# octavian-ganea/equidock_public

Measured on NVIDIA H100. Metric: protein_pairs_per_sec_iegmn_fwd_kabsch, higher is better.
Workload: dtype f32

## Files before the change

### equidock_public_b200/csrc/edge_stage_tc.cu

```cuda
#include "tc_common.cuh"

namespace eqd {
#define TC_WGS 3
#define TC_THREADS (128 * TC_WGS)
#define TC_ROWS 64
#define TC_MAX_TN 32
#define TC_LD 72
#define TC_W_BYTES 67584
#define TC_W1_SPLIT 6144
#define TC_W23_BASE 18432
#define TC_W23_SPLIT 16384
#define TC_HE_FLOATS (TC_ROWS * EQD_EDGE_FEATS + 16)
#define TC_A_SPLIT 6144

struct __align__(128) TcWgSmem {
  unsigned char a[3 * TC_A_SPLIT];
  float msg[TC_ROWS * TC_LD];
  float he[TC_HE_FLOATS];
  double xs[2][TC_ROWS * 6];
  double xm[TC_ROWS * 3];
  double phi[TC_ROWS];
  int src[2][TC_ROWS];
  int dst[2][TC_ROWS];
  int rp[2][TC_MAX_TN + 4];
  unsigned long long he_bar;
};

struct EdgeConsts {
  float ln_g[64], ln_b[64], b2[64], b3[64], w4[64];
};

struct TcSmem {
  unsigned char w[TC_W_BYTES];
  TcWgSmem wg[TC_WGS];
  EdgeConsts cst;
  unsigned long long w_bar;
};

#define TC_CLN_BYTES 512
static_assert(sizeof(TcSmem) + 128 + TC_CLN_BYTES <= 232448, "edge stage shared memory exceeds the sm_90 limit");

template <int P, bool CLN>
__global__ void __launch_bounds__(TC_THREADS, 1)
edge_stage_tc_kernel(eqd_graph g, eqd_layer_params p, const __grid_constant__ EdgeConsts cst_p,
                     const float* __restrict__ proj, const double* __restrict__ x_in, const double* __restrict__ x_orig,
                     float* __restrict__ aggr, double* __restrict__ x_out, int* __restrict__ status, int tn,
                     eqd_layer_norms nm) {
  extern __shared__ __align__(128) unsigned char smem_raw[];
  TcSmem& S = *reinterpret_cast<TcSmem*>(smem_raw);
  float* cln = reinterpret_cast<float*>(smem_raw + sizeof(TcSmem));
  const int tid = threadIdx.x, wgi = tid >> 7, t = tid & 127, r = t & 63, half = t >> 6;
  const int warp = t >> 5, lane = t & 31;
  TcWgSmem& W = S.wg[wgi];
  const EdgeConsts& cst = S.cst;
  const int bar = 1 + wgi;
  const int pw = 128 + 3 * p.dhp;
  const int ntiles = (g.n_nodes + tn - 1) / tn;
  const float slope = p.leaky_slope;

  if (tid == 0) {
    mbar_init(&S.w_bar, 1);
    for (int w = 0; w < TC_WGS; ++w) mbar_init(&S.wg[w].he_bar, 1);
    asm volatile("fence.mbarrier_init.release.cluster;" ::: "memory");
    mbar_expect_tx(&S.w_bar, TC_W_BYTES);
    bulk_g2s(S.w, p.w_edge_tc, TC_W_BYTES, &S.w_bar);
  }
  for (int i = tid; i < 5 * 64; i += TC_THREADS) (&S.cst.ln_g[0])[i] = (&cst_p.ln_g[0])[i];
  if (CLN && tid < 128) cln[tid] = tid < 64 ? nm.coors_ln_g[tid] : nm.coors_ln_b[tid - 64];
  __syncthreads();
  mbar_wait(&S.w_bar, 0);
  unsigned he_phase = 0;
  const unsigned w_saddr = smem_u32(S.w), a_saddr = smem_u32(W.a);
  auto a_desc = [&](int sp, int kb) { return a_desc_at<TC_ROWS>(a_saddr, TC_A_SPLIT, 0, sp, kb); };

  auto prefetch = [&](int tile, int buf, int e0, int e1, int& off_l, int& n_l, int& off_r) {
    const int n0 = tile * tn, nn = min(tn, g.n_nodes - n0);
    const int ne = e1 - e0;
    off_l = off_r = 0;
    n_l = 0;
    if (ne <= TC_ROWS) {
      if (r < ne) {
        if (half == 0) cp_async4(&W.src[buf][r], g.col_src + e0 + r);
        else cp_async4(&W.dst[buf][r], g.edge_dst + e0 + r);
      }
      if (half == 0 && r <= nn) cp_async4(&W.rp[buf][r], g.row_ptr + n0 + r);
      const int el0 = min(e0, g.n_lig_edges), el1 = min(e1, g.n_lig_edges);
      n_l = el1 - el0;
      long sl = 0, sr = 0;
      unsigned bl = 0, br = 0;
      if (n_l > 0) {
        long b0 = (long)el0 * (EQD_EDGE_FEATS * 4), b1 = (long)el1 * (EQD_EDGE_FEATS * 4);
        sl = b0 & ~15L;
        bl = (unsigned)(((b1 + 15) & ~15L) - sl);
        off_l = (int)((b0 - sl) >> 2);
      }
      const int nr = ne - n_l;
      const unsigned dst_r_off = bl;
      if (nr > 0) {
        long b0 = (long)(e0 + n_l - g.n_lig_edges) * (EQD_EDGE_FEATS * 4), b1 = (long)(e1 - g.n_lig_edges) * (EQD_EDGE_FEATS * 4);
        sr = b0 & ~15L;
        br = (unsigned)(((b1 + 15) & ~15L) - sr);
        off_r = (int)(dst_r_off >> 2) + (int)((b0 - sr) >> 2);
      }
      if (t == 0) {
        mbar_expect_tx(&W.he_bar, bl + br);
        if (bl) bulk_g2s(W.he, reinterpret_cast<const unsigned char*>(g.he_lig) + sl, bl, &W.he_bar);
        if (br) bulk_g2s(reinterpret_cast<unsigned char*>(W.he) + dst_r_off, reinterpret_cast<const unsigned char*>(g.he_rec) + sr, br,
                         &W.he_bar);
      }
    }
    cp_async_commit();
  };
  auto prefetch_x = [&](int b, int ne_t) {
    if (r < ne_t && ne_t <= TC_ROWS) {
      const double* xp = x_in + (long)(half == 0 ? W.src[b][r] : W.dst[b][r]) * 3;
#pragma unroll
      for (int c = 0; c < 3; ++c) cp_async8(&W.xs[b][r * 6 + half * 3 + c], xp + c);
    }
    cp_async_commit();
  };
  auto row_range = [&](int tile, int& e0, int& e1) {
    const int n0 = tile * tn;
    e0 = __ldg(g.row_ptr + n0);
    e1 = __ldg(g.row_ptr + n0 + min(tn, g.n_nodes - n0));
  };

  int tile = blockIdx.x * TC_WGS + wgi;
  const int tstride = gridDim.x * TC_WGS;
  int buf = 0;
  int e0 = 0, ne = 0, off_l = 0, n_l = 0, off_r = 0;
  if (tile < ntiles) {
    int e1;
    row_range(tile, e0, e1);
    ne = e1 - e0;
    prefetch(tile, buf, e0, e1, off_l, n_l, off_r);
    cp_async_wait<0>();
    prefetch_x(buf, ne);
  }
  const int fr0 = warp * 16 + (lane >> 2), fc = 2 * (lane & 3);

  for (; tile < ntiles; tile += tstride) {
    const int n0 = tile * tn, nn = min(tn, g.n_nodes - n0);
    const bool has_next = tile + tstride < ntiles;
    int e0n = 0, e1n = 0, off_ln = 0, n_ln = 0, off_rn = 0;
    if (has_next) row_range(tile + tstride, e0n, e1n);
    const int nen = e1n - e0n;
    if (ne > TC_ROWS) {
      if (t == 0) atomicOr(status + g.n_pairs, EQD_STATUS_DEGREE_OVERFLOW);
      cp_async_wait<0>();
      wg_barrier(bar);
      if (has_next) {
        prefetch(tile + tstride, buf ^ 1, e0n, e1n, off_ln, n_ln, off_rn);
        cp_async_wait<0>();
        prefetch_x(buf ^ 1, nen);
      }
      e0 = e0n; ne = nen; off_l = off_ln; n_l = n_ln; off_r = off_rn; buf ^= 1;
      continue;
    }
    const int o_upd = 127 - t;
    const int nd_upd = o_upd / 3, comp_upd = o_upd - nd_upd * 3;
    const long gi_upd = (long)(n0 + nd_upd) * 3 + comp_upd;
    double xo_upd = 0.0, xi_upd = 0.0;
    if (o_upd < nn * 3) {
      xo_upd = x_orig[gi_upd];
      xi_upd = x_in[gi_upd];
    }
    cp_async_wait<0>();
    wg_barrier(bar);
    float2 ps[16], pd[16];
#pragma unroll
    for (int h = 0; h < 2; ++h) {
      const int fr = fr0 + 8 * h;
      const bool ok = fr < ne;
      const float* sp = proj + (long)(ok ? W.src[buf][fr] : 0) * pw + fc;
      const float* dp = proj + (long)(ok ? W.dst[buf][fr] : n0) * pw + 64 + fc;
#pragma unroll
      for (int j = 0; j < 8; ++j) {
        ps[2 * j + h] = __ldg(reinterpret_cast<const float2*>(sp + 8 * j));
        pd[2 * j + h] = __ldg(reinterpret_cast<const float2*>(dp + 8 * j));
      }
    }
    const bool valid = r < ne;
    {
      float a1v[24];
      mbar_wait(&W.he_bar, he_phase);
      he_phase ^= 1;
      const float* hrow = W.he + (r < n_l ? off_l + r * EQD_EDGE_FEATS : off_r + (r - n_l) * EQD_EDGE_FEATS);
      if (half == 0) {
#pragma unroll
        for (int k = 0; k < 24; ++k) a1v[k] = valid ? hrow[k] : 0.f;
      } else {
        double rx = 0.0, ry = 0.0, rz = 0.0;
        if (valid) {
          const double* xs = W.xs[buf] + r * 6;
          rx = xs[0] - xs[3];
          ry = xs[1] - xs[4];
          rz = xs[2] - xs[5];
          W.xm[r * 3 + 0] = rx;
          W.xm[r * 3 + 1] = ry;
          W.xm[r * 3 + 2] = rz;
        }
#pragma unroll
        for (int k = 0; k < 3; ++k) a1v[k] = valid ? hrow[24 + k] : 0.f;
        const float nd2 = valid ? -(float)(rx * rx + ry * ry + rz * rz) : -INFINITY;
        constexpr double kS[EQD_N_RBF] = {1.0, 1.5, 2.25, 3.375, 5.0625, 7.59375, 11.390625, 17.0859375, 25.62890625,
                                          38.443359375, 57.6650390625, 86.49755859375, 129.746337890625,
                                          194.6195068359375, 291.92926025390625};
#pragma unroll
        for (int j = 0; j < EQD_N_RBF; ++j)
          a1v[3 + j] = exp2f(nd2 * (float)(1.4426950408889634 / kS[j]));
#pragma unroll
        for (int k = 18; k < 24; ++k) a1v[k] = 0.f;
      }
      unsigned p0[12], p1[12], p2[12];
#pragma unroll
      for (int c = 0; c < 12; ++c) split3_pair<P>(a1v[2 * c], a1v[2 * c + 1], p0[c], p1[c], p2[c]);
#pragma unroll
      for (int j = 0; j < 3; ++j) a_store8<TC_ROWS, P>(W.a, TC_A_SPLIT, r, half * 24 + 8 * j, p0 + 4 * j, p1 + 4 * j, p2 + 4 * j);
    }
    tc_fence_before();
    const bool deg10 = wg_barrier_and(bar, t >= nn || W.rp[buf][t + 1] - W.rp[buf][t] == 10);
    unsigned af[3][4][4];
    {
      float v[32];
      wg_gemm6_issue<64, 0, P>(v, a_desc, [&](int sp, int kb) { return b_desc_ex(w_saddr + sp * TC_W1_SPLIT + kb * 2048, 1024, 128); },
                         3, false);
      if (has_next) prefetch(tile + tstride, buf ^ 1, e0n, e1n, off_ln, n_ln, off_rn);
      wg_mma_wait(v);
#pragma unroll
      for (int h = 0; h < 2; ++h)
#pragma unroll
        for (int j = 0; j < 8; ++j) {
          float& x0 = v[4 * j + 2 * h];
          float& x1 = v[4 * j + 2 * h + 1];
          x0 = __fadd_rn(__fadd_rn(x0, ps[2 * j + h].x), pd[2 * j + h].x);
          x1 = __fadd_rn(__fadd_rn(x1, ps[2 * j + h].y), pd[2 * j + h].y);
          x0 = fmaxf(x0, __fmul_rn(x0, slope));
          x1 = fmaxf(x1, __fmul_rn(x1, slope));
        }
      float pv[32];
#pragma unroll
      for (int i = 0; i < 32; ++i) pv[i] = __shfl_xor_sync(0xffffffffu, v[i], 2);
      float mean[2], rstd[2];
#pragma unroll
      for (int h = 0; h < 2; ++h) {
        float mh[2], qh[2];
#pragma unroll
        for (int ch = 0; ch < 2; ++ch) {
          float s0 = 0.f, s1 = 0.f;
#pragma unroll
          for (int c4 = 0; c4 < 8; ++c4) {
            s0 = __fadd_rn(s0, chain_val(v, pv, h, ch, c4, 0));
            s1 = __fadd_rn(s1, chain_val(v, pv, h, ch, c4, 1));
          }
          const float sp = s0 + s1;
          mh[ch] = (sp + __shfl_xor_sync(0xffffffffu, sp, 1)) * (1.f / 32.f);
          float q0 = 0.f, q1 = 0.f;
#pragma unroll
          for (int c4 = 0; c4 < 8; ++c4) {
            const float d0 = __fadd_rn(chain_val(v, pv, h, ch, c4, 0), -mh[ch]);
            const float d1 = __fadd_rn(chain_val(v, pv, h, ch, c4, 1), -mh[ch]);
            q0 = fmaf(d0, d0, q0);
            q1 = fmaf(d1, d1, q1);
          }
          const float qp = q0 + q1;
          qh[ch] = qp + __shfl_xor_sync(0xffffffffu, qp, 1);
        }
        const float m0 = mh[0], m1 = mh[1];
        mean[h] = 0.5f * (m0 + m1);
        const float dm = m0 - m1;
        const float var = (qh[0] + qh[1] + dm * dm * 16.f) * (1.f / 64.f);
        rstd[h] = 1.f / sqrtf(var + 1e-5f);
      }
#pragma unroll
      for (int j = 0; j < 8; ++j) {
        const float2 gj = *reinterpret_cast<const float2*>(&cst.ln_g[8 * j + fc]);
        const float2 bj = *reinterpret_cast<const float2*>(&cst.ln_b[8 * j + fc]);
#pragma unroll
        for (int h = 0; h < 2; ++h) {
          float& x0 = v[4 * j + 2 * h];
          float& x1 = v[4 * j + 2 * h + 1];
          x0 = fmaf(__fmul_rn(__fadd_rn(x0, -mean[h]), rstd[h]), gj.x, bj.x);
          x1 = fmaf(__fmul_rn(__fadd_rn(x1, -mean[h]), rstd[h]), gj.y, bj.y);
        }
      }
      acc_to_a_split3<4, P>(v, af);
    }
    if (has_next) {
      cp_async_wait<0>();
      prefetch_x(buf ^ 1, nen);
    }
    {
      auto w23 = [&](int hn) {
        return [&, hn](int sp, int kb) {
          return b_desc_ex(w_saddr + TC_W23_BASE + sp * TC_W23_SPLIT + kb * 4096 + hn * 1024, 2048, 128); };
      };
      float m[32], hd[32];
      wg_gemm6_rs_issue<64, 4, 0, false, P>(m, af, w23(0), false);
      wg_gemm6_rs_issue<64, 4, 0, false, P>(hd, af, w23(1), false);
      wg_mma_wait(m);
      wg_mma_wait(hd);
      float u[32];
#pragma unroll
      for (int j = 0; j < 8; ++j) {
        const float2 b2 = *reinterpret_cast<const float2*>(&cst.b2[8 * j + fc]);
        const float2 b3 = *reinterpret_cast<const float2*>(&cst.b3[8 * j + fc]);
#pragma unroll
        for (int h = 0; h < 2; ++h) {
          *reinterpret_cast<float2*>(W.msg + (fr0 + 8 * h) * TC_LD + 8 * j + fc) =
              make_float2(__fadd_rn(m[4 * j + 2 * h], b2.x), __fadd_rn(m[4 * j + 2 * h + 1], b2.y));
          const float x0 = __fadd_rn(hd[4 * j + 2 * h], b3.x), x1 = __fadd_rn(hd[4 * j + 2 * h + 1], b3.y);
          u[4 * j + 2 * h] = fmaxf(x0, __fmul_rn(x0, slope));
          u[4 * j + 2 * h + 1] = fmaxf(x1, __fmul_rn(x1, slope));
        }
      }
      if (CLN) {
        float mean[2], rstd[2];
        quad_ln_stats(u, mean, rstd);
        quad_ln_apply(u, mean, rstd, cln, cln + 64, fc);
      }
      float pu[32];
#pragma unroll
      for (int i = 0; i < 32; ++i) pu[i] = __shfl_xor_sync(0xffffffffu, u[i], 2);
      double phv[2];
#pragma unroll
      for (int h = 0; h < 2; ++h) {
        double red[2];
#pragma unroll
        for (int ch = 0; ch < 2; ++ch) {
          const float* w4 = cst.w4 + 32 * ch + 2 * (lane & 1);
          float p0 = 0.f, p1 = 0.f;
#pragma unroll
          for (int c4 = 0; c4 < 8; ++c4) {
            p0 = fmaf(chain_val(u, pu, h, ch, c4, 0), w4[4 * c4], p0);
            p1 = fmaf(chain_val(u, pu, h, ch, c4, 1), w4[4 * c4 + 1], p1);
          }
          const double pp = (double)p0 + (double)p1;
          red[ch] = pp + __shfl_xor_sync(0xffffffffu, pp, 1);
        }
        phv[h] = red[0] + red[1] + (double)p.b_coor2;
      }
      if ((lane & 3) == 0) {
        W.phi[fr0] = phv[0];
        W.phi[fr0 + 8] = phv[1];
      }
    }
    wg_barrier(bar);
    if (o_upd < nn * 3) {
      const int rs = W.rp[buf][nd_upd] - e0, re = W.rp[buf][nd_upd + 1] - e0;
      double sum = 0.0;
      if (deg10) {
#pragma unroll
        for (int j = 0; j < 10; ++j) {
          const int rr = nd_upd * 10 + j;
          sum += W.xm[rr * 3 + comp_upd] * W.phi[rr];
        }
      } else {
        for (int rr = rs; rr < re; ++rr) sum += W.xm[rr * 3 + comp_upd] * W.phi[rr];
      }
      const int deg = re - rs;
      const double upd = deg > 0 ? sum / (double)deg : 0.0;
      const double eta = (double)p.x_connection_init;
      x_out[gi_upd] = eta * xo_upd + (1.0 - eta) * xi_upd + upd;
    }
    {
      const int c = t & 63;
      const float* col = W.msg + c;
      if (deg10) {
        for (int nd = (nn * half) >> 1, nd1 = (nn * (half + 1)) >> 1; nd < nd1; ++nd) {
          const float* cr = col + nd * 10 * TC_LD;
          float s0 = 0.f, s1 = 0.f;
#pragma unroll
          for (int j = 0; j < 10; j += 2) {
            s0 += cr[j * TC_LD];
            s1 += cr[(j + 1) * TC_LD];
          }
          aggr[(long)(n0 + nd) * 64 + c] = (s0 + s1) / 10.f;
        }
      } else {
        for (int nd = (nn * half) >> 1, nd1 = (nn * (half + 1)) >> 1; nd < nd1; ++nd) {
          const int rs = W.rp[buf][nd] - e0, re = W.rp[buf][nd + 1] - e0;
          float s0 = 0.f, s1 = 0.f;
          int rr = rs;
          for (; rr + 1 < re; rr += 2) {
            s0 += col[rr * TC_LD];
            s1 += col[(rr + 1) * TC_LD];
          }
          if (rr < re) s0 += col[rr * TC_LD];
          aggr[(long)(n0 + nd) * 64 + c] = re > rs ? (s0 + s1) / (float)(re - rs) : 0.f;
        }
      }
    }
    e0 = e0n; ne = nen; off_l = off_ln; n_l = n_ln; off_r = off_rn; buf ^= 1;
  }
  cp_async_wait<0>();
  __syncthreads();
}

template <int P, bool CLN>
static int launch_edge_stage_tc(const eqd_graph* g, const eqd_layer* p_l, const float* proj, const double* x_in,
                                const double* x_orig, float* aggr, double* x_out, int32_t* status, int tn, void* stream) {
  const int ntiles = (g->n_nodes + tn - 1) / tn;
  EdgeConsts cst;
  memcpy(&cst, p_l->consts.edge, sizeof(cst));
  size_t smem = sizeof(TcSmem) + 128 + (CLN ? TC_CLN_BYTES : 0);
  EQD_SET_SMEM((edge_stage_tc_kernel<P, CLN>), smem);
  int grid = (ntiles + TC_WGS - 1) / TC_WGS;
  if (grid > EQD_SMS) grid = EQD_SMS;
  edge_stage_tc_kernel<P, CLN><<<grid, TC_THREADS, smem, (cudaStream_t)stream>>>(*g, p_l->dev, cst, proj, x_in, x_orig,
                                                                                aggr, x_out, status, tn, p_l->norms);
  EQD_CUDA_LAUNCH_CHECK();
  return EQD_OK;
}

}

extern "C" int eqd_edge_stage(const eqd_graph* g, const eqd_layer* p_l, const float* proj, const double* x_in,
                              const double* x_orig, float* aggr, double* x_out, int32_t* status, void* stream) {
  const eqd_layer_params* p = p_l ? &p_l->dev : nullptr;
  if (!g || !p || !proj || !x_in || !x_orig || !aggr || !x_out || !status) return EQD_ERR_BAD_ARG;
  if (!p->w_edge_tc) return EQD_ERR_BAD_ARG;
  const int cln = eqd_coors_ln(p_l);
  if (cln < 0) return EQD_ERR_BAD_ARG;
  const int products = eqd_mma_products(p);
  if (!products) return EQD_ERR_UNSUPPORTED;
  if (g->max_in_degree < 1 || g->max_in_degree > EQD_TM) return EQD_ERR_UNSUPPORTED;
  if (!(p->leaky_slope >= 0.f && p->leaky_slope <= 1.f)) return EQD_ERR_UNSUPPORTED;
  if ((reinterpret_cast<uintptr_t>(g->he_lig) | reinterpret_cast<uintptr_t>(g->he_rec) |
       reinterpret_cast<uintptr_t>(p->w_edge_tc)) & 15)
    return EQD_ERR_BAD_ARG;
  if (g->max_in_degree > TC_ROWS || p_l->dropout.p > 0.f) return eqd_edge_stage_ffma(g, p_l, proj, x_in, x_orig, aggr, x_out, status, stream);
  if (g->n_nodes <= 0) return EQD_OK;
  int tn = TC_ROWS / g->max_in_degree;
  if (tn > TC_MAX_TN) tn = TC_MAX_TN;
  if (cln)
    return products == 3 ? eqd::launch_edge_stage_tc<3, true>(g, p_l, proj, x_in, x_orig, aggr, x_out, status, tn, stream)
                         : eqd::launch_edge_stage_tc<6, true>(g, p_l, proj, x_in, x_orig, aggr, x_out, status, tn, stream);
  return products == 3 ? eqd::launch_edge_stage_tc<3, false>(g, p_l, proj, x_in, x_orig, aggr, x_out, status, tn, stream)
                       : eqd::launch_edge_stage_tc<6, false>(g, p_l, proj, x_in, x_orig, aggr, x_out, status, tn, stream);
}
```

### equidock_public_b200/csrc/tc_common.cuh

```cuda
#pragma once
#include "common.cuh"

namespace eqd {

__device__ __forceinline__ unsigned smem_u32(const void* p) { return (unsigned)__cvta_generic_to_shared(p); }

__device__ __forceinline__ void mbar_init(unsigned long long* bar, int count) {
  asm volatile("mbarrier.init.shared::cta.b64 [%0], %1;" ::"r"(smem_u32(bar)), "r"(count));
}
__device__ __forceinline__ void mbar_wait(unsigned long long* bar, unsigned parity) {
  unsigned addr = smem_u32(bar);
  unsigned done = 0;
  while (!done) {
    asm volatile(
        "{\n\t.reg .pred p;\n\t"
        "mbarrier.try_wait.parity.shared::cta.b64 p, [%1], %2;\n\t"
        "selp.u32 %0, 1, 0, p;\n\t}"
        : "=r"(done) : "r"(addr), "r"(parity) : "memory");
  }
}
__device__ __forceinline__ void mbar_expect_tx(unsigned long long* bar, unsigned bytes) {
  asm volatile("mbarrier.arrive.expect_tx.shared::cta.b64 _, [%0], %1;" ::"r"(smem_u32(bar)), "r"(bytes) : "memory");
}
__device__ __forceinline__ void bulk_g2s(void* dst, const void* src, unsigned bytes, unsigned long long* bar) {
  asm volatile("cp.async.bulk.shared::cluster.global.mbarrier::complete_tx::bytes [%0], [%1], %2, [%3];" ::"r"(smem_u32(dst)),
               "l"(src), "r"(bytes), "r"(smem_u32(bar)) : "memory");
}
__device__ __forceinline__ void cp_async8(void* dst, const void* src) {
  asm volatile("cp.async.ca.shared.global [%0], [%1], 8;" ::"r"(smem_u32(dst)), "l"(src));
}
__device__ __forceinline__ void cp_async4(void* dst, const void* src) {
  asm volatile("cp.async.ca.shared.global [%0], [%1], 4;" ::"r"(smem_u32(dst)), "l"(src));
}
__device__ __forceinline__ void tc_fence_before() { asm volatile("fence.proxy.async.shared::cta;" ::: "memory"); }

__device__ __forceinline__ unsigned long long b_desc_ex(unsigned saddr, unsigned lbo, unsigned sbo) {
  return (unsigned long long)((saddr >> 4) & 0x3FFF) | ((unsigned long long)((lbo >> 4) & 0x3FFF) << 16) |
         ((unsigned long long)((sbo >> 4) & 0x3FFF) << 32);
}

template <int N, int TB>
struct Wgmma;
template <int TB>
struct Wgmma<16, TB> {
  static __device__ __forceinline__ void mma(float (&d)[8], unsigned long long a, unsigned long long b, int scale_d) {
    asm volatile(
        "{\n\t.reg .pred p;\n\tsetp.ne.b32 p, %10, 0;\n\t"
        "wgmma.mma_async.sync.aligned.m64n16k16.f32.bf16.bf16 {%0, %1, %2, %3, %4, %5, %6, %7}, %8, %9, p, 1, 1, 0, %11;\n\t}"
        : "+f"(d[0]), "+f"(d[1]), "+f"(d[2]), "+f"(d[3]), "+f"(d[4]), "+f"(d[5]), "+f"(d[6]), "+f"(d[7])
        : "l"(a), "l"(b), "r"(scale_d), "n"(TB));
  }
};
template <int TB>
struct Wgmma<64, TB> {
  static __device__ __forceinline__ void mma(float (&d)[32], unsigned long long a, unsigned long long b, int scale_d) {
    asm volatile(
        "{\n\t.reg .pred p;\n\tsetp.ne.b32 p, %34, 0;\n\t"
        "wgmma.mma_async.sync.aligned.m64n64k16.f32.bf16.bf16 {%0, %1, %2, %3, %4, %5, %6, %7, %8, %9, %10, %11, %12, %13, %14, %15, %16, %17, %18, %19, %20, %21, %22, %23, %24, %25, %26, %27, %28, %29, %30, %31}, %32, %33, p, 1, 1, 0, %35;\n\t}"
        : "+f"(d[0]), "+f"(d[1]), "+f"(d[2]), "+f"(d[3]), "+f"(d[4]), "+f"(d[5]), "+f"(d[6]), "+f"(d[7]), "+f"(d[8]), "+f"(d[9]), "+f"(d[10]), "+f"(d[11]), "+f"(d[12]), "+f"(d[13]), "+f"(d[14]), "+f"(d[15]), "+f"(d[16]), "+f"(d[17]), "+f"(d[18]), "+f"(d[19]), "+f"(d[20]), "+f"(d[21]), "+f"(d[22]), "+f"(d[23]), "+f"(d[24]), "+f"(d[25]), "+f"(d[26]), "+f"(d[27]), "+f"(d[28]), "+f"(d[29]), "+f"(d[30]), "+f"(d[31])
        : "l"(a), "l"(b), "r"(scale_d), "n"(TB));
  }
};
template <int TB>
struct Wgmma<80, TB> {
  static __device__ __forceinline__ void mma(float (&d)[40], unsigned long long a, unsigned long long b, int scale_d) {
    asm volatile(
        "{\n\t.reg .pred p;\n\tsetp.ne.b32 p, %42, 0;\n\t"
        "wgmma.mma_async.sync.aligned.m64n80k16.f32.bf16.bf16 {%0, %1, %2, %3, %4, %5, %6, %7, %8, %9, %10, %11, %12, %13, %14, %15, %16, %17, %18, %19, %20, %21, %22, %23, %24, %25, %26, %27, %28, %29, %30, %31, %32, %33, %34, %35, %36, %37, %38, %39}, %40, %41, p, 1, 1, 0, %43;\n\t}"
        : "+f"(d[0]), "+f"(d[1]), "+f"(d[2]), "+f"(d[3]), "+f"(d[4]), "+f"(d[5]), "+f"(d[6]), "+f"(d[7]), "+f"(d[8]), "+f"(d[9]), "+f"(d[10]), "+f"(d[11]), "+f"(d[12]), "+f"(d[13]), "+f"(d[14]), "+f"(d[15]), "+f"(d[16]), "+f"(d[17]), "+f"(d[18]), "+f"(d[19]), "+f"(d[20]), "+f"(d[21]), "+f"(d[22]), "+f"(d[23]), "+f"(d[24]), "+f"(d[25]), "+f"(d[26]), "+f"(d[27]), "+f"(d[28]), "+f"(d[29]), "+f"(d[30]), "+f"(d[31]), "+f"(d[32]), "+f"(d[33]), "+f"(d[34]), "+f"(d[35]), "+f"(d[36]), "+f"(d[37]), "+f"(d[38]), "+f"(d[39])
        : "l"(a), "l"(b), "r"(scale_d), "n"(TB));
  }
};

template <int N, int TB>
struct WgmmaRS;
template <int TB>
struct WgmmaRS<64, TB> {
  static __device__ __forceinline__ void mma(float (&d)[32], const unsigned (&a)[4], unsigned long long b, int scale_d) {
    asm volatile(
        "{\n\t.reg .pred p;\n\tsetp.ne.b32 p, %37, 0;\n\t"
        "wgmma.mma_async.sync.aligned.m64n64k16.f32.bf16.bf16 {%0, %1, %2, %3, %4, %5, %6, %7, %8, %9, %10, %11, %12, %13, %14, %15, %16, %17, %18, %19, %20, %21, %22, %23, %24, %25, %26, %27, %28, %29, %30, %31}, {%32, %33, %34, %35}, %36, p, 1, 1, %38;\n\t}"
        : "+f"(d[0]), "+f"(d[1]), "+f"(d[2]), "+f"(d[3]), "+f"(d[4]), "+f"(d[5]), "+f"(d[6]), "+f"(d[7]), "+f"(d[8]), "+f"(d[9]), "+f"(d[10]), "+f"(d[11]), "+f"(d[12]), "+f"(d[13]), "+f"(d[14]), "+f"(d[15]), "+f"(d[16]), "+f"(d[17]), "+f"(d[18]), "+f"(d[19]), "+f"(d[20]), "+f"(d[21]), "+f"(d[22]), "+f"(d[23]), "+f"(d[24]), "+f"(d[25]), "+f"(d[26]), "+f"(d[27]), "+f"(d[28]), "+f"(d[29]), "+f"(d[30]), "+f"(d[31])
        : "r"(a[0]), "r"(a[1]), "r"(a[2]), "r"(a[3]), "l"(b), "r"(scale_d), "n"(TB));
  }
};

template <int N, int TB = 0, int P = 6, class AD, class BD>
__device__ __forceinline__ void wg_gemm6_issue(float (&d)[N / 2], AD a_desc, BD b_desc, int kblocks, bool accumulate,
                                               bool hi_only = false) {
  static_assert(P == 6 || P == 3, "bf16x6 or bf16x3");
  const int pa[6] = {2, 0, 1, 1, 0, 0}, pb[6] = {0, 2, 1, 0, 1, 0};
  asm volatile("wgmma.fence.sync.aligned;" ::: "memory");
  int scale_d = accumulate ? 1 : 0;
#pragma unroll
  for (int pr = hi_only ? 5 : 6 - P; pr < 6; ++pr)
    for (int kb = 0; kb < kblocks; ++kb) {
      Wgmma<N, TB>::mma(d, a_desc(pa[pr], kb), b_desc(pb[pr], kb), scale_d);
      scale_d = 1;
    }
  asm volatile("wgmma.commit_group.sync.aligned;" ::: "memory");
}
template <int PENDING = 0, int M>
__device__ __forceinline__ void wg_mma_wait(float (&d)[M]) {
  asm volatile("wgmma.wait_group.sync.aligned %0;" ::"n"(PENDING) : "memory");
#pragma unroll
  for (int i = 0; i < M; ++i) asm volatile("" : "+f"(d[i])::"memory");
}
template <int N, int TB = 0, int P = 6, class AD, class BD>
__device__ __forceinline__ void wg_gemm6(float (&d)[N / 2], AD a_desc, BD b_desc, int kblocks, bool accumulate,
                                         bool hi_only = false) {
  wg_gemm6_issue<N, TB, P>(d, a_desc, b_desc, kblocks, accumulate, hi_only);
  asm volatile("wgmma.wait_group.sync.aligned 0;" ::: "memory");
}
template <int N, int KB, int TB = 0, bool HI_ONLY = false, int P = 6, class BD>
__device__ __forceinline__ void wg_gemm6_rs_issue(float (&d)[N / 2], const unsigned (&a)[3][KB][4], BD b_desc, bool accumulate) {
  static_assert(P == 6 || P == 3, "bf16x6 or bf16x3");
  constexpr int pa[6] = {2, 0, 1, 1, 0, 0}, pb[6] = {0, 2, 1, 0, 1, 0};
  asm volatile("wgmma.fence.sync.aligned;" ::: "memory");
  int scale_d = accumulate ? 1 : 0;
#pragma unroll
  for (int pr = HI_ONLY ? 5 : 6 - P; pr < 6; ++pr)
#pragma unroll
    for (int kb = 0; kb < KB; ++kb) {
      WgmmaRS<N, TB>::mma(d, a[pa[pr]][kb], b_desc(pb[pr], kb), scale_d);
      scale_d = 1;
    }
  asm volatile("wgmma.commit_group.sync.aligned;" ::: "memory");
}

template <int R>
__device__ __forceinline__ unsigned long long a_desc_at(unsigned a_saddr, unsigned split_bytes, int wgi, int s, int kb) {
  return b_desc_ex(a_saddr + s * split_bytes + kb * (32 * R) + wgi * 1024, 16 * R, 128);
}
template <int R, int P = 6>
__device__ __forceinline__ void a_store8(unsigned char* a, unsigned split_bytes, int row, int c, const unsigned* p0,
                                         const unsigned* p1, const unsigned* p2) {
  unsigned char* base = a + (c >> 4) * (32 * R) + ((c >> 3) & 1) * (16 * R) + (row >> 3) * 128 + (row & 7) * 16;
  *reinterpret_cast<uint4*>(base) = make_uint4(p0[0], p0[1], p0[2], p0[3]);
  *reinterpret_cast<uint4*>(base + split_bytes) = make_uint4(p1[0], p1[1], p1[2], p1[3]);
  if constexpr (P == 6) *reinterpret_cast<uint4*>(base + 2 * split_bytes) = make_uint4(p2[0], p2[1], p2[2], p2[3]);
}

template <int N>
__device__ __forceinline__ void wg_store_d(float* tile, int ld, const float (&d)[N / 2], int t) {
  const int row = (t >> 5) * 16 + ((t & 31) >> 2), col = 2 * (t & 3);
#pragma unroll
  for (int j = 0; j < N / 8; ++j) {
    *reinterpret_cast<float2*>(tile + row * ld + 8 * j + col) = make_float2(d[4 * j], d[4 * j + 1]);
    *reinterpret_cast<float2*>(tile + (row + 8) * ld + 8 * j + col) = make_float2(d[4 * j + 2], d[4 * j + 3]);
  }
}

__device__ __forceinline__ unsigned cvt_bf16x2(float hi, float lo) {
  unsigned d;
  asm("cvt.rn.bf16x2.f32 %0, %1, %2;" : "=r"(d) : "f"(hi), "f"(lo));
  return d;
}
template <int P = 6>
__device__ __forceinline__ void split3_pair(float v0, float v1, unsigned& p0, unsigned& p1, unsigned& p2) {
  p0 = cvt_bf16x2(v1, v0);
  const float r0 = v0 - __uint_as_float(p0 << 16), r1 = v1 - __uint_as_float(p0 & 0xFFFF0000u);
  p1 = cvt_bf16x2(r1, r0);
  if constexpr (P == 6) p2 = cvt_bf16x2(r1 - __uint_as_float(p1 & 0xFFFF0000u), r0 - __uint_as_float(p1 << 16));
}
template <int R>
__device__ __forceinline__ void store_half_split3(unsigned char* a, unsigned split_bytes, int row, int c0, const float (&v)[32]) {
  unsigned p0[16], p1[16], p2[16];
#pragma unroll
  for (int c = 0; c < 16; ++c) split3_pair(v[2 * c], v[2 * c + 1], p0[c], p1[c], p2[c]);
#pragma unroll
  for (int j = 0; j < 4; ++j) a_store8<R>(a, split_bytes, row, c0 + 8 * j, p0 + 4 * j, p1 + 4 * j, p2 + 4 * j);
}
template <int R>
__device__ __forceinline__ void store_extra8_split3(unsigned char* a, unsigned split_bytes, int row, int c0, const float (&t)[8]) {
  unsigned p0[8], p1[8], p2[8];
#pragma unroll
  for (int c = 0; c < 4; ++c) split3_pair(t[2 * c], t[2 * c + 1], p0[c], p1[c], p2[c]);
#pragma unroll
  for (int c = 4; c < 8; ++c) p0[c] = p1[c] = p2[c] = 0u;
  a_store8<R>(a, split_bytes, row, c0, p0, p1, p2);
  a_store8<R>(a, split_bytes, row, c0 + 8, p0 + 4, p1 + 4, p2 + 4);
}
template <int KB, int P = 6>
__device__ __forceinline__ void acc_to_a_split3(const float (&v)[8 * KB], unsigned (&a)[3][KB][4]) {
#pragma unroll
  for (int kb = 0; kb < KB; ++kb)
#pragma unroll
    for (int i = 0; i < 4; ++i) split3_pair<P>(v[8 * kb + 2 * i], v[8 * kb + 2 * i + 1], a[0][kb][i], a[1][kb][i], a[2][kb][i]);
}
__device__ __forceinline__ int stage_swz(int row) { return (row & 3) << 1; }
__device__ __forceinline__ void stage_rows64(float* rows, const float* src, int ld, int col0, long row0, int nvalid, int t) {
#pragma unroll
  for (int i = 0; i < 8; ++i) {
    const int idx = i * 128 + t, row = idx >> 4, k4 = idx & 15;
    const bool ok = row < nvalid;
    cp_async16(rows + row * 64 + ((k4 ^ stage_swz(row)) << 2), src + (row0 + (ok ? row : 0)) * ld + col0 + 4 * k4, ok);
  }
  cp_async_commit();
}
template <int P = 6>
__device__ __forceinline__ void staged_rows_to_a_split3(const float* rows, int t, unsigned (&a)[3][4][4]) {
  const int g = (t >> 5) * 16 + ((t & 31) >> 2), c = t & 3;
#pragma unroll
  for (int kb = 0; kb < 4; ++kb)
#pragma unroll
    for (int i = 0; i < 4; ++i) {
      const int row = g + 8 * (i & 1), k4 = 4 * kb + 2 * (i >> 1) + (c >> 1);
      const float2 v = *reinterpret_cast<const float2*>(rows + row * 64 + ((k4 ^ stage_swz(row)) << 2) + 2 * (c & 1));
      split3_pair<P>(v.x, v.y, a[0][kb][i], a[1][kb][i], a[2][kb][i]);
    }
}
__device__ __forceinline__ void staged_rows_to_frag(const float* rows, int t, float (&v)[32]) {
  const int g = (t >> 5) * 16 + ((t & 31) >> 2), c = t & 3;
#pragma unroll
  for (int kb = 0; kb < 4; ++kb)
#pragma unroll
    for (int i = 0; i < 4; ++i) {
      const int row = g + 8 * (i & 1), k4 = 4 * kb + 2 * (i >> 1) + (c >> 1);
      const float2 x = *reinterpret_cast<const float2*>(rows + row * 64 + ((k4 ^ stage_swz(row)) << 2) + 2 * (c & 1));
      v[8 * kb + 2 * i] = x.x;
      v[8 * kb + 2 * i + 1] = x.y;
    }
}
__device__ __forceinline__ float chain_val(const float (&v)[32], const float (&pv)[32], int h, int ch, int c4, int e) {
  const int i = 4 * (4 * ch + (c4 >> 1)) + 2 * h + e;
  const bool own = ((c4 & 1) == 0) == ((threadIdx.x & 2) == 0);
  return own ? v[i] : pv[i];
}
__device__ __forceinline__ void wg_barrier(int id) { asm volatile("bar.sync %0, 128;" ::"r"(id) : "memory"); }
__device__ __forceinline__ bool wg_barrier_and(int id, bool pred) {
  unsigned all;
  asm volatile(
      "{\n\t.reg .pred p, q;\n\tsetp.ne.u32 p, %1, 0;\n\t"
      "bar.red.and.pred q, %2, 128, p;\n\tselp.u32 %0, 1, 0, q;\n\t}"
      : "=r"(all) : "r"((unsigned)pred), "r"(id) : "memory");
  return all != 0;
}
__device__ __forceinline__ void tile_ld32f(const float* tile, int ld, int row, int c0, float (&v)[32]) {
  const float4* s = reinterpret_cast<const float4*>(tile + row * ld + c0);
#pragma unroll
  for (int c4 = 0; c4 < 8; ++c4) {
    float4 t = s[c4];
    v[c4 * 4] = t.x; v[c4 * 4 + 1] = t.y; v[c4 * 4 + 2] = t.z; v[c4 * 4 + 3] = t.w;
  }
}

__device__ __forceinline__ void quad_ln_stats(const float (&v)[32], float (&mean)[2], float (&rstd)[2]) {
  float pv[32];
#pragma unroll
  for (int i = 0; i < 32; ++i) pv[i] = __shfl_xor_sync(0xffffffffu, v[i], 2);
#pragma unroll
  for (int h = 0; h < 2; ++h) {
    float mh[2], qh[2];
#pragma unroll
    for (int ch = 0; ch < 2; ++ch) {
      float s0 = 0.f, s1 = 0.f;
#pragma unroll
      for (int c4 = 0; c4 < 8; ++c4) {
        s0 = __fadd_rn(s0, chain_val(v, pv, h, ch, c4, 0));
        s1 = __fadd_rn(s1, chain_val(v, pv, h, ch, c4, 1));
      }
      const float sp = s0 + s1;
      mh[ch] = (sp + __shfl_xor_sync(0xffffffffu, sp, 1)) * (1.f / 32.f);
      float q0 = 0.f, q1 = 0.f;
#pragma unroll
      for (int c4 = 0; c4 < 8; ++c4) {
        const float d0 = __fadd_rn(chain_val(v, pv, h, ch, c4, 0), -mh[ch]);
        const float d1 = __fadd_rn(chain_val(v, pv, h, ch, c4, 1), -mh[ch]);
        q0 = fmaf(d0, d0, q0);
        q1 = fmaf(d1, d1, q1);
      }
      const float qp = q0 + q1;
      qh[ch] = qp + __shfl_xor_sync(0xffffffffu, qp, 1);
    }
    const float m0 = mh[0], m1 = mh[1];
    mean[h] = 0.5f * (m0 + m1);
    const float dm = m0 - m1;
    const float var = (qh[0] + qh[1] + dm * dm * 16.f) * (1.f / 64.f);
    rstd[h] = 1.f / sqrtf(var + 1e-5f);
  }
}

__device__ __forceinline__ void quad_ln_apply(float (&v)[32], const float (&mean)[2], const float (&rstd)[2],
                                              const float* ln_g, const float* ln_b, int fc) {
#pragma unroll
  for (int j = 0; j < 8; ++j) {
    const float2 gj = *reinterpret_cast<const float2*>(&ln_g[8 * j + fc]);
    const float2 bj = *reinterpret_cast<const float2*>(&ln_b[8 * j + fc]);
#pragma unroll
    for (int h = 0; h < 2; ++h) {
      float& x0 = v[4 * j + 2 * h];
      float& x1 = v[4 * j + 2 * h + 1];
      x0 = fmaf(__fmul_rn(__fadd_rn(x0, -mean[h]), rstd[h]), gj.x, bj.x);
      x1 = fmaf(__fmul_rn(__fadd_rn(x1, -mean[h]), rstd[h]), gj.y, bj.y);
    }
  }
}

}
```

Measured before the change: 43200.

## Build first edge GEMM operand in registers and merge message/hidden GEMMs

Each thread now builds the first-layer A operand (edge features plus RBF expansion) directly in the register-fragment layout and feeds it to register-sourced wgmma, so the shared-memory A staging buffer, its stores and the async-proxy fence go away. The two second-layer GEMMs are merged into a single m64n128 wgmma. Global loads of projections and coordinates are moved to overlap with the outstanding MMAs. Register pressure rises (64-float accumulator plus A fragments), and the RBF values are computed redundantly across the four threads of each quad, which could cause spills or extra ALU work.

```diff
diff --git a/equidock_public_b200/csrc/edge_stage_tc.cu b/equidock_public_b200/csrc/edge_stage_tc.cu
--- a/equidock_public_b200/csrc/edge_stage_tc.cu
+++ b/equidock_public_b200/csrc/edge_stage_tc.cu
@@ -11,10 +11,8 @@
 #define TC_W23_BASE 18432
 #define TC_W23_SPLIT 16384
 #define TC_HE_FLOATS (TC_ROWS * EQD_EDGE_FEATS + 16)
-#define TC_A_SPLIT 6144
 
 struct __align__(128) TcWgSmem {
-  unsigned char a[3 * TC_A_SPLIT];
   float msg[TC_ROWS * TC_LD];
   float he[TC_HE_FLOATS];
   double xs[2][TC_ROWS * 6];
@@ -39,6 +37,13 @@
 
 #define TC_CLN_BYTES 512
 static_assert(sizeof(TcSmem) + 128 + TC_CLN_BYTES <= 232448, "edge stage shared memory exceeds the sm_90 limit");
+
+__host__ __device__ constexpr float rbf_scale(int j) {
+  constexpr double kS[EQD_N_RBF] = {1.0, 1.5, 2.25, 3.375, 5.0625, 7.59375, 11.390625, 17.0859375, 25.62890625,
+                                    38.443359375, 57.6650390625, 86.49755859375, 129.746337890625,
+                                    194.6195068359375, 291.92926025390625};
+  return (float)(1.4426950408889634 / kS[j]);
+}
 
 template <int P, bool CLN>
 __global__ void __launch_bounds__(TC_THREADS, 1)
@@ -70,8 +75,7 @@
   __syncthreads();
   mbar_wait(&S.w_bar, 0);
   unsigned he_phase = 0;
-  const unsigned w_saddr = smem_u32(S.w), a_saddr = smem_u32(W.a);
-  auto a_desc = [&](int sp, int kb) { return a_desc_at<TC_ROWS>(a_saddr, TC_A_SPLIT, 0, sp, kb); };
+  const unsigned w_saddr = smem_u32(S.w);
 
   auto prefetch = [&](int tile, int buf, int e0, int e1, int& off_l, int& n_l, int& off_r) {
     const int n0 = tile * tn, nn = min(tn, g.n_nodes - n0);
@@ -161,72 +165,73 @@
     const int nd_upd = o_upd / 3, comp_upd = o_upd - nd_upd * 3;
     const long gi_upd = (long)(n0 + nd_upd) * 3 + comp_upd;
     double xo_upd = 0.0, xi_upd = 0.0;
-    if (o_upd < nn * 3) {
-      xo_upd = x_orig[gi_upd];
-      xi_upd = x_in[gi_upd];
-    }
     cp_async_wait<0>();
     wg_barrier(bar);
-    float2 ps[16], pd[16];
+    unsigned a1[3][3][4];
+    mbar_wait(&W.he_bar, he_phase);
+    he_phase ^= 1;
 #pragma unroll
     for (int h = 0; h < 2; ++h) {
       const int fr = fr0 + 8 * h;
-      const bool ok = fr < ne;
-      const float* sp = proj + (long)(ok ? W.src[buf][fr] : 0) * pw + fc;
-      const float* dp = proj + (long)(ok ? W.dst[buf][fr] : n0) * pw + 64 + fc;
-#pragma unroll
-      for (int j = 0; j < 8; ++j) {
-        ps[2 * j + h] = __ldg(reinterpret_cast<const float2*>(sp + 8 * j));
-        pd[2 * j + h] = __ldg(reinterpret_cast<const float2*>(dp + 8 * j));
-      }
-    }
-    const bool valid = r < ne;
-    {
-      float a1v[24];
-      mbar_wait(&W.he_bar, he_phase);
-      he_phase ^= 1;
-      const float* hrow = W.he + (r < n_l ? off_l + r * EQD_EDGE_FEATS : off_r + (r - n_l) * EQD_EDGE_FEATS);
-      if (half == 0) {
-#pragma unroll
-        for (int k = 0; k < 24; ++k) a1v[k] = valid ? hrow[k] : 0.f;
-      } else {
-        double rx = 0.0, ry = 0.0, rz = 0.0;
-        if (valid) {
-          const double* xs = W.xs[buf] + r * 6;
-          rx = xs[0] - xs[3];
-          ry = xs[1] - xs[4];
-          rz = xs[2] - xs[5];
-          W.xm[r * 3 + 0] = rx;
-          W.xm[r * 3 + 1] = ry;
-          W.xm[r * 3 + 2] = rz;
-        }
-#pragma unroll
-        for (int k = 0; k < 3; ++k) a1v[k] = valid ? hrow[24 + k] : 0.f;
-        const float nd2 = valid ? -(float)(rx * rx + ry * ry + rz * rz) : -INFINITY;
-        constexpr double kS[EQD_N_RBF] = {1.0, 1.5, 2.25, 3.375, 5.0625, 7.59375, 11.390625, 17.0859375, 25.62890625,
-                                          38.443359375, 57.6650390625, 86.49755859375, 129.746337890625,
-                                          194.6195068359375, 291.92926025390625};
-#pragma unroll
-        for (int j = 0; j < EQD_N_RBF; ++j)
-          a1v[3 + j] = exp2f(nd2 * (float)(1.4426950408889634 / kS[j]));
-#pragma unroll
-        for (int k = 18; k < 24; ++k) a1v[k] = 0.f;
-      }
-      unsigned p0[12], p1[12], p2[12];
-#pragma unroll
-      for (int c = 0; c < 12; ++c) split3_pair<P>(a1v[2 * c], a1v[2 * c + 1], p0[c], p1[c], p2[c]);
-#pragma unroll
-      for (int j = 0; j < 3; ++j) a_store8<TC_ROWS, P>(W.a, TC_A_SPLIT, r, half * 24 + 8 * j, p0 + 4 * j, p1 + 4 * j, p2 + 4 * j);
-    }
-    tc_fence_before();
+      const bool valid = fr < ne;
+      const float* hrow = W.he + (fr < n_l ? off_l + fr * EQD_EDGE_FEATS : off_r + (fr - n_l) * EQD_EDGE_FEATS);
+      double rx = 0.0, ry = 0.0, rz = 0.0;
+      if (valid) {
+        const double* xs = W.xs[buf] + fr * 6;
+        rx = xs[0] - xs[3];
+        ry = xs[1] - xs[4];
+        rz = xs[2] - xs[5];
+        if (fc == 0) {
+          W.xm[fr * 3 + 0] = rx;
+          W.xm[fr * 3 + 1] = ry;
+          W.xm[fr * 3 + 2] = rz;
+        }
+      }
+      const float nd2 = valid ? -(float)(rx * rx + ry * ry + rz * rz) : -INFINITY;
+      auto rbf = [&](int j0) {
+        auto sc = [](int j) { return rbf_scale(min(max(j, 0), EQD_N_RBF - 1)); };
+        const float s = fc == 0 ? sc(j0) : fc == 2 ? sc(j0 + 2) : fc == 4 ? sc(j0 + 4) : sc(j0 + 6);
+        return exp2f(nd2 * s);
+      };
+#pragma unroll
+      for (int kb = 0; kb < 3; ++kb)
+#pragma unroll
+        for (int ih = 0; ih < 2; ++ih) {
+          const int c0 = 16 * kb + 8 * ih;
+          float x[2];
+#pragma unroll
+          for (int e = 0; e < 2; ++e) {
+            const int col = c0 + fc + e;
+            if (c0 < 24) x[e] = valid ? hrow[col] : 0.f;
+            else if (c0 == 24) x[e] = col < EQD_EDGE_FEATS ? (valid ? hrow[col] : 0.f) : rbf(c0 + e - EQD_EDGE_FEATS);
+            else if (c0 == 32) x[e] = rbf(c0 + e - EQD_EDGE_FEATS);
+            else x[e] = fc == 0 ? rbf(c0 + e - EQD_EDGE_FEATS) : 0.f;
+          }
+          split3_pair<P>(x[0], x[1], a1[0][kb][2 * ih + h], a1[1][kb][2 * ih + h], a1[2][kb][2 * ih + h]);
+        }
+    }
     const bool deg10 = wg_barrier_and(bar, t >= nn || W.rp[buf][t + 1] - W.rp[buf][t] == 10);
     unsigned af[3][4][4];
     {
       float v[32];
-      wg_gemm6_issue<64, 0, P>(v, a_desc, [&](int sp, int kb) { return b_desc_ex(w_saddr + sp * TC_W1_SPLIT + kb * 2048, 1024, 128); },
-                         3, false);
+      wg_gemm6_rs_issue<64, 3, 0, false, P>(v, a1, [&](int sp, int kb) {
+        return b_desc_ex(w_saddr + sp * TC_W1_SPLIT + kb * 2048, 1024, 128); }, false);
+      float2 ps[16], pd[16];
+#pragma unroll
+      for (int h = 0; h < 2; ++h) {
+        const int fr = fr0 + 8 * h;
+        const bool ok = fr < ne;
+        const float* sp = proj + (long)(ok ? W.src[buf][fr] : 0) * pw + fc;
+        const float* dp = proj + (long)(ok ? W.dst[buf][fr] : n0) * pw + 64 + fc;
+#pragma unroll
+        for (int j = 0; j < 8; ++j) {
+          ps[2 * j + h] = __ldg(reinterpret_cast<const float2*>(sp + 8 * j));
+          pd[2 * j + h] = __ldg(reinterpret_cast<const float2*>(dp + 8 * j));
+        }
+      }
       if (has_next) prefetch(tile + tstride, buf ^ 1, e0n, e1n, off_ln, n_ln, off_rn);
       wg_mma_wait(v);
+      wg_rs_release<P>(a1);
 #pragma unroll
       for (int h = 0; h < 2; ++h)
 #pragma unroll
@@ -286,20 +291,20 @@
       }
       acc_to_a_split3<4, P>(v, af);
     }
-    if (has_next) {
-      cp_async_wait<0>();
-      prefetch_x(buf ^ 1, nen);
-    }
     {
-      auto w23 = [&](int hn) {
-        return [&, hn](int sp, int kb) {
-          return b_desc_ex(w_saddr + TC_W23_BASE + sp * TC_W23_SPLIT + kb * 4096 + hn * 1024, 2048, 128); };
-      };
-      float m[32], hd[32];
-      wg_gemm6_rs_issue<64, 4, 0, false, P>(m, af, w23(0), false);
-      wg_gemm6_rs_issue<64, 4, 0, false, P>(hd, af, w23(1), false);
-      wg_mma_wait(m);
-      wg_mma_wait(hd);
+      float mh[64];
+      wg_gemm6_rs_issue<128, 4, 0, false, P>(mh, af, [&](int sp, int kb) {
+        return b_desc_ex(w_saddr + TC_W23_BASE + sp * TC_W23_SPLIT + kb * 4096, 2048, 128); }, false);
+      if (has_next) {
+        cp_async_wait<0>();
+        prefetch_x(buf ^ 1, nen);
+      }
+      if (o_upd < nn * 3) {
+        xo_upd = x_orig[gi_upd];
+        xi_upd = x_in[gi_upd];
+      }
+      wg_mma_wait(mh);
+      wg_rs_release<P>(af);
       float u[32];
 #pragma unroll
       for (int j = 0; j < 8; ++j) {
@@ -308,8 +313,8 @@
 #pragma unroll
         for (int h = 0; h < 2; ++h) {
           *reinterpret_cast<float2*>(W.msg + (fr0 + 8 * h) * TC_LD + 8 * j + fc) =
-              make_float2(__fadd_rn(m[4 * j + 2 * h], b2.x), __fadd_rn(m[4 * j + 2 * h + 1], b2.y));
-          const float x0 = __fadd_rn(hd[4 * j + 2 * h], b3.x), x1 = __fadd_rn(hd[4 * j + 2 * h + 1], b3.y);
+              make_float2(__fadd_rn(mh[4 * j + 2 * h], b2.x), __fadd_rn(mh[4 * j + 2 * h + 1], b2.y));
+          const float x0 = __fadd_rn(mh[32 + 4 * j + 2 * h], b3.x), x1 = __fadd_rn(mh[32 + 4 * j + 2 * h + 1], b3.y);
           u[4 * j + 2 * h] = fmaxf(x0, __fmul_rn(x0, slope));
           u[4 * j + 2 * h + 1] = fmaxf(x1, __fmul_rn(x1, slope));
         }
diff --git a/equidock_public_b200/csrc/tc_common.cuh b/equidock_public_b200/csrc/tc_common.cuh
--- a/equidock_public_b200/csrc/tc_common.cuh
+++ b/equidock_public_b200/csrc/tc_common.cuh
@@ -81,6 +81,16 @@
         "{\n\t.reg .pred p;\n\tsetp.ne.b32 p, %37, 0;\n\t"
         "wgmma.mma_async.sync.aligned.m64n64k16.f32.bf16.bf16 {%0, %1, %2, %3, %4, %5, %6, %7, %8, %9, %10, %11, %12, %13, %14, %15, %16, %17, %18, %19, %20, %21, %22, %23, %24, %25, %26, %27, %28, %29, %30, %31}, {%32, %33, %34, %35}, %36, p, 1, 1, %38;\n\t}"
         : "+f"(d[0]), "+f"(d[1]), "+f"(d[2]), "+f"(d[3]), "+f"(d[4]), "+f"(d[5]), "+f"(d[6]), "+f"(d[7]), "+f"(d[8]), "+f"(d[9]), "+f"(d[10]), "+f"(d[11]), "+f"(d[12]), "+f"(d[13]), "+f"(d[14]), "+f"(d[15]), "+f"(d[16]), "+f"(d[17]), "+f"(d[18]), "+f"(d[19]), "+f"(d[20]), "+f"(d[21]), "+f"(d[22]), "+f"(d[23]), "+f"(d[24]), "+f"(d[25]), "+f"(d[26]), "+f"(d[27]), "+f"(d[28]), "+f"(d[29]), "+f"(d[30]), "+f"(d[31])
+        : "r"(a[0]), "r"(a[1]), "r"(a[2]), "r"(a[3]), "l"(b), "r"(scale_d), "n"(TB));
+  }
+};
+template <int TB>
+struct WgmmaRS<128, TB> {
+  static __device__ __forceinline__ void mma(float (&d)[64], const unsigned (&a)[4], unsigned long long b, int scale_d) {
+    asm volatile(
+        "{\n\t.reg .pred p;\n\tsetp.ne.b32 p, %69, 0;\n\t"
+        "wgmma.mma_async.sync.aligned.m64n128k16.f32.bf16.bf16 {%0, %1, %2, %3, %4, %5, %6, %7, %8, %9, %10, %11, %12, %13, %14, %15, %16, %17, %18, %19, %20, %21, %22, %23, %24, %25, %26, %27, %28, %29, %30, %31, %32, %33, %34, %35, %36, %37, %38, %39, %40, %41, %42, %43, %44, %45, %46, %47, %48, %49, %50, %51, %52, %53, %54, %55, %56, %57, %58, %59, %60, %61, %62, %63}, {%64, %65, %66, %67}, %68, p, 1, 1, %70;\n\t}"
+        : "+f"(d[0]), "+f"(d[1]), "+f"(d[2]), "+f"(d[3]), "+f"(d[4]), "+f"(d[5]), "+f"(d[6]), "+f"(d[7]), "+f"(d[8]), "+f"(d[9]), "+f"(d[10]), "+f"(d[11]), "+f"(d[12]), "+f"(d[13]), "+f"(d[14]), "+f"(d[15]), "+f"(d[16]), "+f"(d[17]), "+f"(d[18]), "+f"(d[19]), "+f"(d[20]), "+f"(d[21]), "+f"(d[22]), "+f"(d[23]), "+f"(d[24]), "+f"(d[25]), "+f"(d[26]), "+f"(d[27]), "+f"(d[28]), "+f"(d[29]), "+f"(d[30]), "+f"(d[31]), "+f"(d[32]), "+f"(d[33]), "+f"(d[34]), "+f"(d[35]), "+f"(d[36]), "+f"(d[37]), "+f"(d[38]), "+f"(d[39]), "+f"(d[40]), "+f"(d[41]), "+f"(d[42]), "+f"(d[43]), "+f"(d[44]), "+f"(d[45]), "+f"(d[46]), "+f"(d[47]), "+f"(d[48]), "+f"(d[49]), "+f"(d[50]), "+f"(d[51]), "+f"(d[52]), "+f"(d[53]), "+f"(d[54]), "+f"(d[55]), "+f"(d[56]), "+f"(d[57]), "+f"(d[58]), "+f"(d[59]), "+f"(d[60]), "+f"(d[61]), "+f"(d[62]), "+f"(d[63])
         : "r"(a[0]), "r"(a[1]), "r"(a[2]), "r"(a[3]), "l"(b), "r"(scale_d), "n"(TB));
   }
 };
@@ -126,6 +136,15 @@
       scale_d = 1;
     }
   asm volatile("wgmma.commit_group.sync.aligned;" ::: "memory");
+}
+template <int P = 6, int KB>
+__device__ __forceinline__ void wg_rs_release(const unsigned (&a)[3][KB][4]) {
+#pragma unroll
+  for (int s = 0; s < (P == 6 ? 3 : 2); ++s)
+#pragma unroll
+    for (int kb = 0; kb < KB; ++kb)
+#pragma unroll
+      for (int i = 0; i < 4; ++i) asm volatile("" ::"r"(a[s][kb][i]) : "memory");
 }
 
 template <int R>
```

Measured after the change: 44080, median of 6. +2.0%, better.
